# dog-qiuqiu/Yolo-FastestV2

Hardware: AMD Instinct MI355X
Metric: images/sec at 352x352 bs=256 per GPU (forward+decode+NMS) (higher is better)
Workload: dtype f32 tensors; contractions fp16x3 (two-term fp16 split operands on v_mfma_f32_16x16x32_f16, fp32 accumulate); depthwise/BN/ReLU/decode/NMS fp32 VALU; 1 GPU

## Files before the change

yolo_fastestv2_amd/csrc/yfv2_api.hip:

```cpp
#include <algorithm>
#include <cstdio>

#include "yfv2_ctx.h"

void read_plan_switches(yfv2_ctx* h, const yfv2_plan* plan) {
  h->sw.plan = read_sized(plan);
  h->sw.bf6 = !h->sw.plan.fp32_matrix;
  h->postfuse = !h->sw.plan.post_two_launches;
  h->sw.front_wanted = !h->sw.plan.front_two_launches;
}

int run_plan(yfv2_ctx* h, const void* x, bool x_u8, int B, float* const out6[6], hipStream_t stream, hipEvent_t* ev, int only_step) {
  const RunCtx c{h->d_params, x, x_u8, B, out6, stream, h->sw.bf6, h->nonfinite.dev};
  std::string err;
  if (int rc = plan_run(h->plan, c, h->d_trace, h->trace_step, ev, only_step, &err)) return fail(h, rc, err);
  if (only_step < 0) { h->last_x = x; h->last_B = B; h->last_u8 = x_u8; }
  HIP_TRY(h, hipGetLastError());
  return YFV2_OK;
}

int check_call(yfv2_ctx* h, int B, bool need_weights) {
  if (!h) return fail(nullptr, YFV2_ERR_ARG, "null handle");
  if (B < 1 || B > h->cfg.max_batch)
    return fail(h, YFV2_ERR_BATCH, "batch " + std::to_string(B) + " outside [1, max_batch=" + std::to_string(h->cfg.max_batch) + "]");
  if (need_weights && !h->weights_loaded) return fail(h, YFV2_ERR_STATE, "yfv2_load_weights has not been called");
  return YFV2_OK;
}

int check_config(const yfv2_config* cfg, int* rows_out) {
  if (cfg->anchor_num != 3)
    return fail(nullptr, YFV2_ERR_CONFIG, "anchor_num must be 3 (the reference decode hard-codes 3 anchors per scale)");
  if (cfg->classes < 1 || cfg->classes > 255)
    return fail(nullptr, YFV2_ERR_CONFIG, "classes must be in [1, 255]");
  if (cfg->height < 32 || cfg->width < 32 || cfg->height % 32 || cfg->width % 32)
    return fail(nullptr, YFV2_ERR_CONFIG, "height/width must be multiples of 32");
  if (cfg->max_batch < 1) return fail(nullptr, YFV2_ERR_CONFIG, "max_batch must be >= 1");
  const long long rows_ll = 3LL * ((long long)(cfg->height / 16) * (cfg->width / 16) + (long long)(cfg->height / 32) * (cfg->width / 32));
  if (rows_ll > yfv2_nms_max_rows())
    return fail(nullptr, YFV2_ERR_CONFIG, "more than " + std::to_string(yfv2_nms_max_rows()) + " decode rows per image (" + std::to_string(rows_ll) +
                                          ": inputs beyond 512x512) is not supported by the NMS kernel");
  const int rows = (int)rows_ll;
  *rows_out = rows;
  return YFV2_OK;
}

namespace {

thread_local std::string g_tls_error;
thread_local bool g_creating_lane = false;

int alloc_buf(yfv2_ctx* h, Buf* b, size_t per_img) {
  b->per_img = per_img;
  HIP_TRY(h, hipMalloc(reinterpret_cast<void**>(&b->p), per_img * sizeof(float) * (size_t)h->cfg.max_batch));
  return YFV2_OK;
}

void free_buf(Buf* b) {
  if (b->p) (void)hipFree(b->p);
  b->p = nullptr;
}

size_t logit_elems(const yfv2_ctx* h, int i) { return logit_elems(h->cfg, i); }

constexpr int LANES_DEFAULT = 1, LANES_MAX = 8, LANE_MIN_IMAGES = 32;

int create_lanes(yfv2_ctx* h) {
  int n = h->sw.plan.lanes > 1 ? h->sw.plan.lanes : LANES_DEFAULT;
  if (h->d_trace || h->in_lane) n = 1;
  n = n < 1 ? 1 : (n > LANES_MAX ? LANES_MAX : n);
  if (n == 1 || h->cfg.max_batch < n * LANE_MIN_IMAGES) return YFV2_OK;
  h->lane_min = n * LANE_MIN_IMAGES;
  yfv2_config c = h->cfg;
  c.max_batch = (h->cfg.max_batch + n - 1) / n;
  for (int i = 0; i < n; ++i) {
    yfv2_ctx* lane = nullptr;
    yfv2_plan lp = h->sw.plan;
    lp.lanes = 0; lp.trace = 0;
    g_creating_lane = true;
    const int rc = yfv2_create_ex(&lane, &c, &lp);
    g_creating_lane = false;
    if (rc) return fail(h, rc, "lane " + std::to_string(i) + ": " + g_tls_error);
    lane->nonfinite.dev = h->nonfinite.dev;
    h->lanes.push_back(lane);
  }
  HIP_TRY(h, hipEventCreateWithFlags(&h->lane_fork, hipEventDisableTiming));
  for (int i = 1; i < n; ++i) {
    hipStream_t st; hipEvent_t ev;
    HIP_TRY(h, hipStreamCreateWithFlags(&st, hipStreamNonBlocking));
    h->lane_stream.push_back(st);
    HIP_TRY(h, hipEventCreateWithFlags(&ev, hipEventDisableTiming));
    h->lane_join.push_back(ev);
  }
  return YFV2_OK;
}

template <class F>
int run_lanes(yfv2_ctx* h, int B, hipStream_t s, F f) {
  const int n = (int)h->lanes.size();
  const int per = (B + n - 1) / n;
  h->last_split.clear();
  h->last_x = nullptr; h->last_B = 0;
  HIP_TRY(h, hipEventRecord(h->lane_fork, s));
  int rc = YFV2_OK;
  auto hip_ok = [&](hipError_t e, const char* what) {
    if (e != hipSuccess && rc == YFV2_OK) rc = fail(h, YFV2_ERR_DEVICE, std::string(what) + ": " + hipGetErrorString(e));
    return e == hipSuccess;
  };
  std::vector<char> forked((size_t)n, 0);
  for (int i = 1; i < n && rc == YFV2_OK; ++i) {
    const int off = i * per, cnt = std::min(per, B - off);
    if (cnt <= 0) break;
    if (!hip_ok(hipStreamWaitEvent(h->lane_stream[i - 1], h->lane_fork, 0), "hipStreamWaitEvent(lane fork)")) break;
    forked[(size_t)i] = 1;
    const int lrc = f(h->lanes[i], off, cnt, h->lane_stream[i - 1]);
    if (lrc) { rc = lrc; h->err = h->lanes[i]->err; }
  }
  if (rc == YFV2_OK) {
    rc = f(h->lanes[0], 0, std::min(per, B), s);
    if (rc) h->err = h->lanes[0]->err;
  }
  for (int i = 1; i < n; ++i) {
    if (!forked[(size_t)i]) continue;
    if (hip_ok(hipEventRecord(h->lane_join[i - 1], h->lane_stream[i - 1]), "hipEventRecord(lane join)"))
      hip_ok(hipStreamWaitEvent(s, h->lane_join[i - 1], 0), "hipStreamWaitEvent(lane join)");
    else
      (void)hipStreamSynchronize(h->lane_stream[i - 1]);
  }
  if (rc == YFV2_OK)
    for (int i = 0; i < n; ++i) { const int cnt = std::min(per, B - i * per); if (cnt > 0) h->last_split.push_back(cnt); }
  return rc;
}

bool use_lanes(const yfv2_ctx* h, int B) { return !h->lanes.empty() && B >= h->lane_min; }

}

int build_plan(yfv2_ctx* h, WeightPacker& wp, const yfv2_tensor_desc* tensors, int32_t n, yfv2_ctx* report) {
  h->plan = Plan{};
  if (!wp.index(h->cfg, tensors, n)) return fail(report, YFV2_ERR_WEIGHTS, wp.missing);
  if (!plan_build(h->cfg, h->sw, h->ws, wp, &h->plan)) return fail(report, YFV2_ERR_WEIGHTS, "weight packing failed");
  return YFV2_OK;
}

void** yfv2_ctx_train_slot(yfv2_ctx* h) { return h ? &h->train : nullptr; }
const yfv2_config* yfv2_ctx_config(yfv2_ctx* h) { return &h->cfg; }
int yfv2_ctx_fail(yfv2_ctx* h, int code, const char* msg) {
  g_tls_error = msg ? msg : "";
  if (h) h->err = g_tls_error;
  return code;
}

DecodeArgs decode_args(yfv2_ctx* h, const float* const out6[6], int32_t B) {
  DecodeArgs a{};
  for (int sc = 0; sc < 2; ++sc) {
    a.reg[sc] = out6[sc * 3 + 0];
    a.obj[sc] = out6[sc * 3 + 1];
    a.cls[sc] = out6[sc * 3 + 2];
    a.fh[sc] = h->fh[sc];
    a.fw[sc] = h->fw[sc];
    a.stride[sc] = (float)((double)h->cfg.height / (double)h->fh[sc]);
  }
  for (int i = 0; i < 12; ++i) a.anchors[i] = h->cfg.anchors[i];
  a.B = B;
  a.classes = h->cfg.classes;
  a.rows = h->rows;
  return a;
}

NmsArgs nms_args(const yfv2_ctx* h, const float* boxes, int compact, int32_t B, float conf_thres, double iou_thres, float* dets, int32_t* idx, int32_t* count) {
  NmsArgs a{};
  a.boxes = boxes; a.compact = compact; a.dets = dets; a.idx = idx; a.count = count;
  a.B = B; a.rows = h->rows; a.nc = h->cfg.classes;
  a.conf_thres = conf_thres; a.iou_thres = iou_thres;
  return a;
}

static const void* image_at(const yfv2_ctx* h, const void* x, bool x_u8, int off) {
  return static_cast<const char*>(x) + (size_t)off * 3 * h->cfg.height * h->cfg.width * (x_u8 ? 1 : sizeof(float));
}

extern "C" {

int yfv2_abi_version(void) { return YFV2_ABI_VERSION; }

const char* yfv2_last_error(yfv2_handle h) { return h ? h->err.c_str() : g_tls_error.c_str(); }

int yfv2_create(yfv2_handle* out, const yfv2_config* cfg) { return yfv2_create_ex(out, cfg, nullptr); }

int yfv2_create_ex(yfv2_handle* out, const yfv2_config* cfg, const yfv2_plan* plan) {
  if (!out || !cfg) return fail(nullptr, YFV2_ERR_ARG, "yfv2_create: null argument");
  *out = nullptr;
  int rows = 0;
  if (int rc = check_config(cfg, &rows)) return rc;

  int ndev = 0;
  if (hipGetDeviceCount(&ndev) != hipSuccess || ndev <= 0 || cfg->device < 0 || cfg->device >= ndev)
    return fail(nullptr, YFV2_ERR_DEVICE, "no usable HIP device (this library has no CPU fallback)");
  hipDeviceProp_t prop;
  if (hipGetDeviceProperties(&prop, cfg->device) != hipSuccess)
    return fail(nullptr, YFV2_ERR_DEVICE, "hipGetDeviceProperties failed");
  if (std::strncmp(prop.gcnArchName, "gfx950", 6) != 0)
    return fail(nullptr, YFV2_ERR_DEVICE, std::string("device is ") + prop.gcnArchName + ", this library is built for gfx950 (MI355X) only");

  yfv2_ctx* h = new yfv2_ctx();
  h->in_lane = g_creating_lane;
  DeviceGuard guard(cfg->device);
  int rc = setup_ctx(h, cfg, rows, alloc_buf);
  if (rc == YFV2_OK && hipMalloc(reinterpret_cast<void**>(&h->d_classes), 258 * sizeof(int32_t)) != hipSuccess)
    rc = fail(h, YFV2_ERR_DEVICE, "hipMalloc(class filter) failed");
  if (rc == YFV2_OK && hipMalloc(reinterpret_cast<void**>(&h->d_frames), sizeof(ResizeFrame) * (size_t)cfg->max_batch) != hipSuccess)
    rc = fail(h, YFV2_ERR_DEVICE, "hipMalloc(frame table) failed");
  if (rc == YFV2_OK) {
    h->d_stats_flag = h->d_classes + 256;
    if (hipMemset(h->d_stats_flag, 0, 2 * sizeof(int32_t)) != hipSuccess) rc = fail(h, YFV2_ERR_DEVICE, "hipMemset(flags) failed");
  }
  if (rc == YFV2_OK && !h->in_lane) {
    if (!h->nonfinite.alloc()) rc = fail(h, YFV2_ERR_DEVICE, "hipHostMalloc(range-guard word) failed");
    else *reinterpret_cast<volatile int32_t*>(h->nonfinite.host) = 0;
  }
  if (rc != YFV2_OK) {
    g_tls_error = h->err;
    yfv2_destroy(h);
    return rc;
  }
  read_plan_switches(h, plan);
  if (h->sw.plan.trace) {
    h->trace_step = h->sw.plan.trace_step;
    (void)hipMalloc(reinterpret_cast<void**>(&h->d_trace), 8192 * sizeof(long long));
    (void)hipMemset(h->d_trace, 0, 8192 * sizeof(long long));
  }
  if (int rc2 = create_lanes(h)) { g_tls_error = h->err; yfv2_destroy(h); return rc2; }
  *out = h;
  return YFV2_OK;
}

void yfv2_destroy(yfv2_handle h) {
  if (!h) return;
  DeviceGuard guard(h->device);
  h->ws.for_each(h->cfg, h->rows, [](Buf& b, size_t) { free_buf(&b); });
  if (h->d_classes) (void)hipFree(h->d_classes);
  if (h->d_frames) (void)hipFree(h->d_frames);
  if (h->d_probe) (void)hipFree(h->d_probe);
  if (h->train) { yfv2_train_release(h->train); h->train = nullptr; }
  if (h->d_params) (void)hipFree(h->d_params);
  for (yfv2_ctx* lane : h->lanes) yfv2_destroy(lane);
  for (hipStream_t st : h->lane_stream) { (void)hipStreamSynchronize(st); (void)hipStreamDestroy(st); }
  for (hipEvent_t ev : h->lane_join) (void)hipEventDestroy(ev);
  if (h->lane_fork) (void)hipEventDestroy(h->lane_fork);
  delete h;
}

int yfv2_load_weights(yfv2_handle h, const yfv2_tensor_desc* tensors, int32_t n) {
  if (!h) return fail(nullptr, YFV2_ERR_ARG, "null handle");
  if (!tensors || n <= 0) return fail(h, YFV2_ERR_ARG, "yfv2_load_weights: no tensors");
  DeviceGuard guard(h->device);
  WeightPacker wp;
  if (int rc = build_plan(h, wp, tensors, n, h)) {
    h->weights_loaded = false;
    return rc;
  }
  HIP_TRY(h, hipDeviceSynchronize());
  if (h->d_params && h->n_params < wp.blob.size()) { (void)hipFree(h->d_params); h->d_params = nullptr; }
  if (!h->d_params) {
    HIP_TRY(h, hipMalloc(reinterpret_cast<void**>(&h->d_params), wp.blob.size() * sizeof(float)));
    h->n_params = wp.blob.size();
  }
  HIP_TRY(h, hipMemcpy(h->d_params, wp.blob.data(), wp.blob.size() * sizeof(float), hipMemcpyHostToDevice));
  h->weights_loaded = true;
  for (yfv2_ctx* lane : h->lanes)
    if (int rc = yfv2_load_weights(lane, tensors, n)) { h->weights_loaded = false; return fail(h, rc, lane->err); }
  return YFV2_OK;
}

int yfv2_set_anchors(yfv2_handle h, const double anchors[12]) {
  if (!h) return fail(nullptr, YFV2_ERR_ARG, "null handle");
  if (!anchors) return fail(h, YFV2_ERR_ARG, "yfv2_set_anchors: null pointer");
  for (int i = 0; i < 12; ++i) h->cfg.anchors[i] = anchors[i];
  for (yfv2_ctx* lane : h->lanes) (void)yfv2_set_anchors(lane, anchors);
  return YFV2_OK;
}

static int forward_impl(yfv2_handle h, const void* x, bool x_u8, int32_t B, float* const out6[6], void* stream) {
  const std::string name = x_u8 ? "yfv2_forward_u8" : "yfv2_forward";
  int rc = check_call(h, B, true);
  if (rc) return rc;
  if (!x || !out6) return fail(h, YFV2_ERR_ARG, name + ": null pointer");
  for (int i = 0; i < 6; ++i)
    if (!out6[i]) return fail(h, YFV2_ERR_ARG, name + ": null output tensor");
  DeviceGuard guard(h->device);
  if (use_lanes(h, B))
    return run_lanes(h, B, static_cast<hipStream_t>(stream), [&](yfv2_ctx* lane, int off, int cnt, hipStream_t st) {
      float* o6[6];
      for (int i = 0; i < 6; ++i) o6[i] = out6[i] + (size_t)off * logit_elems(h, i);
      return forward_impl(lane, image_at(h, x, x_u8, off), x_u8, cnt, o6, st);
    });
  h->last_split.clear();
  return run_plan(h, x, x_u8, B, out6, static_cast<hipStream_t>(stream), nullptr);
}
int yfv2_forward(yfv2_handle h, const float* x, int32_t B, float* const out6[6], void* stream) { return forward_impl(h, x, false, B, out6, stream); }
int yfv2_forward_u8(yfv2_handle h, const uint8_t* x, int32_t B, float* const out6[6], void* stream) { return forward_impl(h, x, true, B, out6, stream); }

static int post_impl(yfv2_handle h, const float* const out6[6], int32_t B, float conf_thres, double iou_thres, float* dets, int32_t* idx,
                     int32_t* count, void* stream);
static int decode_impl(yfv2_handle h, const float* const out6[6], int32_t B, float* boxes, float* cand, void* stream);
static int nms_impl(yfv2_handle h, const float* boxes, int compact, int32_t B, float conf_thres, double iou_thres,
                    const int32_t* classes, int32_t n_classes, float* dets, int32_t* idx, int32_t* count, void* stream);

int yfv2_decode(yfv2_handle h, const float* const out6[6], int32_t B, float* boxes, void* stream) {
  return decode_impl(h, out6, B, boxes, nullptr, stream);
}

static int decode_impl(yfv2_handle h, const float* const out6[6], int32_t B, float* boxes, float* cand, void* stream) {
  int rc = check_call(h, B, false);
  if (rc) return rc;
  if (!out6 || (!boxes && !cand)) return fail(h, YFV2_ERR_ARG, "yfv2_decode: null pointer");
  for (int i = 0; i < 6; ++i)
    if (!out6[i]) return fail(h, YFV2_ERR_ARG, "yfv2_decode: null logit tensor");
  DeviceGuard guard(h->device);
  DecodeArgs a = decode_args(h, out6, B);
  a.boxes = boxes;
  a.cand = cand;
  yfv2_launch_decode(a, static_cast<hipStream_t>(stream));
  HIP_TRY(h, hipGetLastError());
  return YFV2_OK;
}

// ... 121 lines not shown
```

yolo_fastestv2_amd/csrc/yfv2_internal.h:

```cpp
#pragma once
#include <hip/hip_runtime.h>
#include <hip/hip_ext.h>
#include <stdint.h>

typedef float f32x4 __attribute__((ext_vector_type(4)));
typedef float f32x2 __attribute__((ext_vector_type(2)));
typedef float f32x3u __attribute__((ext_vector_type(3), aligned(4)));
typedef unsigned int u32x2 __attribute__((ext_vector_type(2)));
typedef unsigned int u32x3 __attribute__((ext_vector_type(3)));

#ifdef __HIPCC__
__device__ __forceinline__ int yfv2_fdiv(int n, float inv_d) { return (int)(((float)n + 0.5f) * inv_d); }
#endif

#include <atomic>

struct Yfv2LaunchProbe { hipEvent_t start = nullptr, stop = nullptr; int launches = 0; };
extern thread_local Yfv2LaunchProbe yfv2_launch_probe;
#define YFV2_LAUNCH(kernel, grid, block, lds, stream, ...)                                                                        \
  do {                                                                                                                             \
    Yfv2LaunchProbe& yfv2_lp_ = yfv2_launch_probe;                                                                                 \
    hipExtLaunchKernelGGL(kernel, grid, block, lds, stream, yfv2_lp_.launches++ == 0 ? yfv2_lp_.start : nullptr, yfv2_lp_.stop, 0, \
                          __VA_ARGS__);                                                                                            \
  } while (0)
// ... 99 lines not shown
  int relu;
  float* copy;
  int copy_stride;
  int copy_off;
  int H, W;
  int HW;
  float* nchw0;
  float* nchw1;
  int split;
  int ctot0, coff0;
  int bf6;
  int presplit;
  int* nonfinite;
};

struct DwArgs {
  const float* in;
  float* out;
  const float* w;
  const float* scale;
  const float* shift;
  int B, H, W, C;
  int OH, OW;
  int in_stride, in_off;
  int out_stride, out_off;
  int relu;
};

struct BlockS1Args {
  const float* in;
  float* out;
  const float* img;
  long long* trace;
  int B, H, W;
  int R;
  int nblk;
  int presplit;
  int* nonfinite;
  float* park;
};

bool yfv2_s1chain_supported(int c2, int H, int W);
int yfv2_s1chain_image_floats();
long yfv2_s1chain_park_floats(int H, int W, int nblk);
bool yfv2_launch_block_s1chain(const BlockS1Args& a, hipStream_t s);
bool yfv2_s1pool_supported(int c2, int H, int W);
int yfv2_s1pool_image_floats(bool presplit);
bool yfv2_launch_block_s1pool(const BlockS1Args& a, hipStream_t s);

struct BlockS2Args {
  const float* in;
  float* out;
  const float* img;
  int B, H, W;
  int R;
  int s4_main_bands;
  int pp_in;
  unsigned pp_mask;
  long long pp_bufstride;
  long long pp_imgstride;
  int bf6;
  long long* trace;
  const float* img16;
  int* nonfinite;
};
bool yfv2_s3h_supported(int H, int W);
void yfv2_launch_s3h(const BlockS2Args& a, hipStream_t s);
bool yfv2_s4h_supported(int H, int W);
void yfv2_launch_s4h(const BlockS2Args& a, hipStream_t s);

__host__ __device__ inline int yfv2_stage2_channel(int slot) {
  const int p = slot >> 1, e = slot & 1;
  const int b0 = p / 12, b1 = (p % 12) / 6, b2 = (p % 6) / 3, h = 2 * (p % 3) + e;
  return b0 + 2 * b1 + 4 * b2 + 8 * h;
}
struct S1PxArgs {
  float* act;
  const float* img;
  int B, H, W;
  int nstrips, nb, R;
  int img_stride;
  int num_records;
  int src_off[12];
  int dst_off[12];
  const float* img16;
  int* nonfinite;
};
struct S2PxArgs {
  const float* in;
  float* act;
  const float* img[2];
  int B, IH, IW;
  int nstrips, nb, R;
  int in_stride, out_stride;
  int in_records, out_records;
  int st2_off[2][8];
  int st1_off[2][8];
  const float* img16;
  int* nonfinite;
};
struct FrontArgs {
  const void* x;
  int H, W;
  int u8_in;
  const float* img_stem;
  S2PxArgs s2;
};
void yfv2_launch_front(const FrontArgs& a, hipStream_t s);
void yfv2_launch_s2px(const S2PxArgs& a, hipStream_t s);
void yfv2_launch_s2h(const S2PxArgs& a, hipStream_t s);
bool yfv2_s1px_supported(int H, int W);
void yfv2_launch_s1px(const S1PxArgs& a, hipStream_t s);
void yfv2_launch_s1h(const S1PxArgs& a, hipStream_t s);

struct TowerArgs {
  const float* in;
  float* out;
  const float* img;
  int has_head;
  int mh, split;
  float* nchw0; float* nchw1;
  int B, H, W;
  long long* trace;
  int bf6;
  const float* img16;
  int chain;
  int* nonfinite;
};

struct DecodeArgs {
  const float* reg[2];
  const float* obj[2];
  const float* cls[2];
  float* boxes;
  float* cand;
  int B, classes;
  int fh[2], fw[2];
  float stride[2];
  double anchors[12];
  int rows;
};

struct NmsArgs {
  const float* boxes;
  int compact;
  float* dets;
  int32_t* idx;
  int32_t* count;
  const int32_t* classes;
  int n_classes;
  int B, rows, nc;
  float conf_thres;
  double iou_thres;
  long long* trace;
};

void yfv2_launch_stem(const StemArgs& a, hipStream_t s);
void yfv2_launch_stem16(const StemArgs& a, hipStream_t s);
bool yfv2_launch_pw(int K, int mode, const PwArgs& a, hipStream_t s);
int yfv2_pw_tiles(int K, int mode, int M);
bool yfv2_pw_presplit_supported(int K, int mode, int M);
bool yfv2_launch_dw(int ksize, int stride, const DwArgs& a, hipStream_t s);
int yfv2_block_s2_rows(int cin, int H, int W);
bool yfv2_launch_block_s2(int cin, const BlockS2Args& a, hipStream_t s);
bool yfv2_tower2_supported(int H, int W);
bool yfv2_launch_tower2(const TowerArgs& a, hipStream_t s);
bool yfv2_towerh_supported(int H, int W);
bool yfv2_towerh_multi(int H, int W);
struct TowerJobs {
  TowerArgs j[4];
  int n;
  int par;
  int gpj;
  unsigned char lane_patch[128];
};
bool yfv2_launch_towerh(const TowerJobs& jobs, int mh_tiles, hipStream_t s);
struct StatsArgs {
  const float* dets;
  const int32_t* count;
  const float* targets;
  int32_t* tp;
  int32_t* overflow;
  int B, T;
  float iou_thres;
};
constexpr int STATS_MAX_TARGETS = 1024;
void yfv2_launch_stats(const StatsArgs& a, hipStream_t s);
struct StatsMultiArgs {
  const float* dets; const int32_t* count; const float* targets;
  uint32_t* tpmask;
  int32_t* overflow;
  int B, T, K;
  float thr[32];
};
void yfv2_launch_stats_multi(const StatsMultiArgs& a, hipStream_t s);
struct LossMatch {
  int valid, b, a, gj, gi, cls;
  float tb[4];
  double aw, ah;
};
struct LossArgs {
  const float* reg[2]; const float* obj[2]; const float* cls[2];
  float* grad_reg[2]; float* grad_obj[2]; float* grad_cls[2];
  const float* targets;
  LossMatch* matches;
  unsigned char* tobj[2];
  int* nb;
  double* sums;
  float* losses;
  int B, T, classes;
  int fh[2], fw[2];
  double stride[2];
  double anchors[12];
};
void yfv2_launch_loss(const LossArgs& a, hipStream_t s);
struct ResizeArgs {
  const unsigned char* src;
  unsigned char* dst;
  int B, SH, SW, H, W;
  double scale_x, scale_y;
};
size_t yfv2_resize_lds_bytes(int SW, int W);
void yfv2_launch_resize(const ResizeArgs& a, hipStream_t s);
struct ResizeFrame {
  const unsigned char* data;
  long long pitch;
  int h, w;
  double scale_x, scale_y;
  double box_x, box_y;
};
void yfv2_launch_resize_frames(const ResizeFrame* frames, int B, int max_w, unsigned char* dst, int H, int W, hipStream_t s);
void yfv2_launch_frame_boxes(float* dets, const int32_t* count, const ResizeFrame* frames, int B, hipStream_t s);
void yfv2_launch_decode(const DecodeArgs& a, hipStream_t s);
void yfv2_launch_nms(const NmsArgs& a, hipStream_t s);
void yfv2_launch_decode_nms(const DecodeArgs& d, const NmsArgs& a, hipStream_t s);
bool yfv2_post_fusable(int classes, int rows);
int yfv2_nms_max_rows();
struct TileMergeArgs {
  const float* tile_dets;
  const int32_t* tile_count;
  const int32_t* table;
  int T, F;
  float* geo;
  float* meta;
  double thres;
  int metric;
  int max_out;
  float* dets;
  int32_t* src;
  int32_t* count;
};
void yfv2_launch_tile_merge(const TileMergeArgs& a, hipStream_t s);
constexpr int YFV2_KM_CH = 1024;
constexpr int YFV2_KM_MAXK = 32;
struct KmArgs {
  const double* wh;
  int64_t N;
  double* centroids;
  int k;
  int64_t nchunks;
  int32_t* assign;
  double* avg_iou;
  double* part_sum;
  int* part_cnt;
  int* part_flag;
  int* done;
  int32_t* host_word;
};
void yfv2_launch_km_pass(const KmArgs& a, int pass, int last, hipStream_t s);
constexpr int YFV2_AP_CH = 1024;
constexpr int YFV2_AP_TILE = 2048;
struct ApHead {
  long long n_gt[256], n_pred[256];
  double p[256], r[256], ap[256];
  int32_t bad, pad;
};
struct ApArgs {
  const int32_t* tp; const float* conf; const float* pred_cls;
  const uint32_t* tpmask;
  int K;
  int64_t N;
  const float* target_cls;
  int64_t T;
  uint32_t* key[2];
  uint32_t* val[2];
  uint32_t* hist;
  uint32_t* tot;
  double* part;
  int64_t part_stride;
  uint32_t* pmask;
  ApHead* head;
  int nblk;
};
size_t yfv2_ap_ws_bytes(int64_t N, int K);
void yfv2_ap_carve(ApArgs& a, char* ws);
void yfv2_launch_ap(const ApArgs& a, hipStream_t s);
struct yfv2_ap_result;
void yfv2_ap_finish(const ApHead& head, yfv2_ap_result* out);
void yfv2_ap_finish_multi(ApHead* heads, int K, yfv2_ap_result* out);
struct ClockProbeArgs {
  unsigned long long* out;
  unsigned long long ref_ticks;
  int busy;
};
bool yfv2_launch_clock_probe(const ClockProbeArgs& a, int workgroups, hipStream_t s);

struct yfv2_ctx;
struct yfv2_config;
// ... 5 lines not shown
```

yolo_fastestv2_amd/csrc/yfv2_post.hip:

```cpp
#include "yfv2_internal.h"

__device__ __forceinline__ float sigmoid_f32(float x) { return __fdiv_rn(1.0f, __fadd_rn(1.0f, expf(-x))); }

template <int J>
__device__ __forceinline__ int quad_xor(int v) {
  static_assert(J == 1 || J == 2, "quad_perm exchange inside four lanes");
  return __builtin_amdgcn_update_dpp(0, v, J == 1 ? 0xB1 : 0x4E, 0xF, 0xF, false);
}
template <int J> __device__ __forceinline__ float quad_xor(float v) { return __int_as_float(quad_xor<J>(__float_as_int(v))); }

template <bool SKIP = false, int MAXPER = 24>
__device__ __forceinline__ void yfv2_compact_row(const DecodeArgs& a, int b, int sc, int cc, int part, f32x4& r0, f32x4& r1,
                                                 float objl = 0.f, float skip_ct = 0.f) {
  const int fh = a.fh[sc], fw = a.fw[sc], hw = fh * fw;
  const int nc = a.classes;
  const int per = (nc + 3) >> 2;
  const int c_lo = part * per, c_hi = min(nc, c_lo + per);
  const int an = part < 3 ? part : 0;
  const float* cls = a.cls[sc] + (size_t)b * nc * hw;
  const float so = sigmoid_f32(SKIP ? objl : a.obj[sc][((size_t)b * 3 + an) * hw + cc]);
  float conf = 0.f;
  int cj = 0;
  int need = 1;
  if constexpr (SKIP) {
// ... 176 lines not shown
        if (c < c_hi) {
          srow[5 + c] = ev[i];
          srow[rowlen + 5 + c] = ev[i];
          srow[2 * rowlen + 5 + c] = ev[i];
        }
      }
      if (part < 3) {
        float o[5];
        box_of(part, o);
        float* d = srow + part * rowlen;
#pragma unroll
        for (int k = 0; k < 5; ++k) d[k] = o[k];
      }
    }
    __syncthreads();
    float* dst = a.boxes + row0 * rowlen;
    const int n = ncell * 3 * rowlen;
    for (int i = tid; i < n; i += THREADS) dst[i] = stage[i];
  }
}

void yfv2_launch_decode(const DecodeArgs& a, hipStream_t s) {
  const int cells = a.classes <= 96 ? DEC_CELLS : 32;
  const int b0 = (a.fh[0] * a.fw[0] + cells - 1) / cells;
  const int b1 = (a.fh[1] * a.fw[1] + cells - 1) / cells;
  const size_t lds = (size_t)cells * 3 * (5 + a.classes) * sizeof(float);
  static std::atomic<unsigned long long> lds_ok0{0}, lds_ok1{0}, lds_ok2{0}, lds_ok3{0};
  if (a.classes <= 96) {
    yfv2_allow_full_lds(reinterpret_cast<const void*>(&decode_kernel<false>), lds_ok0);
    yfv2_allow_full_lds(reinterpret_cast<const void*>(&decode_kernel<true>), lds_ok1);
    if (a.cand)
      YFV2_LAUNCH(decode_kernel<true>, dim3(a.B * (b0 + b1)), dim3(DEC_THREADS), 0, s, a, b0, b1);
    else
      YFV2_LAUNCH(decode_kernel<false>, dim3(a.B * (b0 + b1)), dim3(DEC_THREADS), lds, s, a, b0, b1);
  } else {
    yfv2_allow_full_lds(reinterpret_cast<const void*>(&decode_kernel<false, 64>), lds_ok2);
    yfv2_allow_full_lds(reinterpret_cast<const void*>(&decode_kernel<true, 64>), lds_ok3);
    if (a.cand)
      YFV2_LAUNCH((decode_kernel<true, 64>), dim3(a.B * (b0 + b1)), dim3(4 * cells), 0, s, a, b0, b1);
    else
      YFV2_LAUNCH((decode_kernel<false, 64>), dim3(a.B * (b0 + b1)), dim3(4 * cells), lds, s, a, b0, b1);
  }
}
bool yfv2_post_fusable(int classes, int rows) { return classes <= 96 && rows <= 2048; }
int yfv2_nms_max_rows() { return 4096; }

constexpr int NMS_THREADS = 1024;
constexpr int NMS_NQ = NMS_THREADS / 64;
constexpr int NMS_CAP = 2048;
constexpr int NMS_MAX_DET = 300;

__device__ __forceinline__ unsigned xor_sel_mask() {
  const int l = (int)(threadIdx.x & 63);
  const bool s4 = __builtin_amdgcn_update_dpp(0, l, 0x124, 0xF, 0xF, false) == (l ^ 4);
  const auto p16 = __builtin_amdgcn_permlane16_swap(l, l, false, false);
  const auto p32 = __builtin_amdgcn_permlane32_swap(l, l, false, false);
  return (s4 ? 4u : 0u) | ((int)p16[0] == (l ^ 16) ? 16u : 0u) | ((int)p32[0] == (l ^ 32) ? 32u : 0u);
}
template <int J>
__device__ __forceinline__ unsigned xor_lane32(unsigned v, unsigned sel) {
  const int x = (int)v;
  if constexpr (J == 1 || J == 2) return (unsigned)quad_xor<J>(x);
  else if constexpr (J == 8) return (unsigned)__builtin_amdgcn_update_dpp(0, x, 0x128, 0xF, 0xF, false);
  else if constexpr (J == 4) {
    const int r4 = __builtin_amdgcn_update_dpp(0, x, 0x124, 0xF, 0xF, false), r12 = __builtin_amdgcn_update_dpp(0, x, 0x12C, 0xF, 0xF, false);
    return (unsigned)((sel & 4u) ? r4 : r12);
  } else if constexpr (J == 16) {
    const auto p = __builtin_amdgcn_permlane16_swap(x, x, false, false);
    return (unsigned)((sel & 16u) ? (int)p[0] : (int)p[1]);
  } else {
    static_assert(J == 32, "lane distance");
    const auto p = __builtin_amdgcn_permlane32_swap(x, x, false, false);
    return (unsigned)((sel & 32u) ? (int)p[0] : (int)p[1]);
  }
}
template <int J>
__device__ __forceinline__ unsigned long long xor_lane64(unsigned long long v, unsigned sel) {
  return ((unsigned long long)xor_lane32<J>((unsigned)(v >> 32), sel) << 32) | xor_lane32<J>((unsigned)v, sel);
}

template <int KPT>
__device__ __forceinline__ void bitonic_sort(unsigned long long* key, unsigned long long* key2, int np2, int tid) {
  const unsigned sel = xor_sel_mask();
  unsigned long long k[KPT];
#pragma unroll
  for (int r = 0; r < KPT; ++r) { const int i = tid + r * NMS_THREADS; k[r] = i < np2 ? key[i] : 0ull; }
  auto cx = [](unsigned long long x, unsigned long long y, bool take_max) { return take_max == (x > y) ? x : y; };
  int pb = 0;
  for (int kk = 2; kk <= np2; kk <<= 1) {
    int j = kk >> 1;
    for (; j >= 64; j >>= 1) {
      if (j >= NMS_THREADS) {
        const int jr = j / NMS_THREADS;
#pragma unroll
        for (int r = 0; r < KPT; ++r) {
          if ((r & jr) == 0 && (r | jr) < KPT) {
            const int r2 = r | jr;
            const bool desc = ((tid + r * NMS_THREADS) & kk) == 0;
            const unsigned long long hi = k[r] > k[r2] ? k[r] : k[r2], lo = k[r] > k[r2] ? k[r2] : k[r];
            k[r] = desc ? hi : lo; k[r2] = desc ? lo : hi;
          }
        }
      } else {
        unsigned long long* buf = pb ? key2 : key;
#pragma unroll
        for (int r = 0; r < KPT; ++r) buf[tid + r * NMS_THREADS] = k[r];
        __syncthreads();
        const bool low = (tid & j) == 0;
#pragma unroll
        for (int r = 0; r < KPT; ++r) {
          const int i = tid + r * NMS_THREADS;
          k[r] = cx(k[r], buf[i ^ j], low == ((i & kk) == 0));
        }
        pb ^= 1;
      }
    }
#define YFV2_SORT_STEP(J)                                                                   \
    if (J < kk) {                                                                           \
      const bool low = (tid & J) == 0;                                                      \
      _Pragma("unroll") for (int r = 0; r < KPT; ++r) {                                     \
        const int i = tid + r * NMS_THREADS;                                                \
        k[r] = cx(k[r], xor_lane64<J>(k[r], sel), low == ((i & kk) == 0));                 \
      }                                                                                     \
    }
    YFV2_SORT_STEP(32) YFV2_SORT_STEP(16) YFV2_SORT_STEP(8) YFV2_SORT_STEP(4) YFV2_SORT_STEP(2) YFV2_SORT_STEP(1)
#undef YFV2_SORT_STEP
  }
  __syncthreads();
#pragma unroll
  for (int r = 0; r < KPT; ++r) { const int i = tid + r * NMS_THREADS; if (i < np2) key[i] = k[r]; }
  __syncthreads();
}

__device__ __forceinline__ unsigned conf_key(float c) {
  const unsigned u = __float_as_uint(c == 0.f ? 0.f : c);
  return (u & 0x80000000u) ? ~u : (u | 0x80000000u);
}

#define NMS_STAMP(i) do { if (a.trace && blockIdx.x == 0 && threadIdx.x == 0) a.trace[i] = (long long)__builtin_readcyclecounter(); } while (0)
template <int SRC, int KPT = 2>
__global__ __launch_bounds__(NMS_THREADS) void nms_kernel(NmsArgs a, DecodeArgs dec) {
  constexpr bool COMPACT = SRC >= 1;
  constexpr int CAP = KPT * NMS_THREADS;
  static_assert(KPT == 2 || (KPT == 4 && SRC != 2), "two keys per thread, or four without the in-LDS decode");
  extern __shared__ __attribute__((aligned(16))) float crow[];
  __shared__ unsigned long long key[CAP];
  __shared__ __attribute__((aligned(16))) float geo[(KPT == 2 ? 7 : 5) * CAP];
  unsigned long long* const key2 = reinterpret_cast<unsigned long long*>(geo);
  float* const bx1 = geo + (KPT == 2 ? 2 * CAP : 0);
  float* const by1 = bx1 + CAP; float* const bx2 = by1 + CAP; float* const by2 = bx2 + CAP; float* const area = by2 + CAP;
  __shared__ unsigned char supp[CAP];
  __shared__ unsigned char cls_of_row[CAP];
  __shared__ int keep[NMS_MAX_DET];
  __shared__ float kx1[NMS_MAX_DET], kx2[NMS_MAX_DET];
  __shared__ unsigned long long pmask[NMS_NQ][64];
  __shared__ int n_cand, n_keep, n_obj;

  const int tid = threadIdx.x, b = blockIdx.x;
  const int rowlen = COMPACT ? 8 : 5 + a.nc;
  const float* img = SRC == 2 ? crow : a.boxes + (size_t)b * a.rows * rowlen;
  const float ct = a.conf_thres;
  NMS_STAMP(0);
  if constexpr (SRC == 2) {
    constexpr int WC = 16;
    const int hw0 = dec.fh[0] * dec.fw[0], hw1 = dec.fh[1] * dec.fw[1];
    const int nw0 = (hw0 + WC - 1) / WC, nw = nw0 + (hw1 + WC - 1) / WC;
    const int wv = __builtin_amdgcn_readfirstlane(tid >> 6);
    const int part = tid & 3, an = part < 3 ? part : 0;
    auto obj_of = [&](int w) -> float {
      if (w >= nw) return 0.f;
      const int sc = w >= nw0 ? 1 : 0, hw = sc ? hw1 : hw0;
      const int cell = (w - (sc ? nw0 : 0)) * WC + ((tid & 63) >> 2);
      return dec.obj[sc][((size_t)b * 3 + an) * hw + (cell < hw ? cell : hw - 1)];
    };
    float ocur = obj_of(wv);
    for (int w = wv; w < nw; w += NMS_NQ) {
      const float onxt = obj_of(w + NMS_NQ);
      const int sc = w >= nw0 ? 1 : 0, hw = sc ? hw1 : hw0;
      const int row_base = sc ? 3 * hw0 : 0;
      const int cell = (w - (sc ? nw0 : 0)) * WC + ((tid & 63) >> 2);
      const bool ok = cell < hw;
      f32x4 r0, r1;
      yfv2_compact_row<true>(dec, b, sc, ok ? cell : hw - 1, part, r0, r1, ocur, ct);
      if (ok && part < 3) {
        float* d = crow + (size_t)(row_base + cell * 3 + part) * 8;
        *reinterpret_cast<f32x4*>(d) = r0;
        *reinterpret_cast<f32x4*>(d + 4) = r1;
      }
      ocur = onxt;
    }
    __syncthreads();
  }
  NMS_STAMP(1);
  unsigned short* cand_row = reinterpret_cast<unsigned short*>(bx1);
  if (tid == 0) { n_cand = 0; n_keep = 0; n_obj = 0; }
  __syncthreads();

  if constexpr (COMPACT) {
    for (int n0 = 0; n0 < a.rows; n0 += NMS_THREADS) {
      const int n = n0 + tid;
      f32x4 t = {0.f, 0.f, 0.f, 0.f};
      if (n < a.rows) t = *reinterpret_cast<const f32x4*>(img + (size_t)n * 8 + 4);
      const bool pass = n < a.rows && t[0] > ct && t[1] > ct;
      const unsigned long long m = __ballot(pass);
      int base = 0;
      if ((tid & 63) == 0 && m) base = atomicAdd(&n_cand, (int)__popcll(m));
      base = __shfl(base, 0);
      if (pass) {
        const int slot = base + (int)__popcll(m & ((1ull << (tid & 63)) - 1ull));
        key[slot] = ((unsigned long long)conf_key(t[1]) << 32) | (unsigned long long)(0xFFFFFFFFu - (unsigned)n);
        cls_of_row[n] = (unsigned char)(int)t[2];
      }
    }
  } else {
    for (int n0 = 0; n0 < a.rows; n0 += NMS_THREADS) {
      const int n = n0 + tid;
      const bool pass = n < a.rows && img[(size_t)n * rowlen + 4] > ct;
      const unsigned long long m = __ballot(pass);
      int base = 0;
      if ((tid & 63) == 0 && m) base = atomicAdd(&n_obj, (int)__popcll(m));
      base = __shfl(base, 0);
      if (pass) cand_row[base + (int)__popcll(m & ((1ull << (tid & 63)) - 1ull))] = (unsigned short)n;
    }
    __syncthreads();
    {
      const int l16 = tid & 15, grp = tid >> 4, ngrp = NMS_THREADS >> 4;
      const int nobj = n_obj;
      for (int q = grp; q < nobj; q += ngrp) {
        const int n = cand_row[q];
        const float* r = img + (size_t)n * rowlen;
        const float obj = r[4];
        float best = -INFINITY;
        int bj = 0x7fffffff;
        for (int j = l16; j < a.nc; j += 16) {
          const float pj = __fmul_rn(r[5 + j], obj);
          if (pj > best || (pj != pj && best == best)) { best = pj; bj = j; }
        }
#pragma unroll
        for (int m = 1; m < 16; m <<= 1) {
          const float ob = __shfl_xor(best, m, 16);
          const int oj = __shfl_xor(bj, m, 16);
          const bool take = ob != ob ? (best == best || oj < bj) : (best == best && (ob > best || (ob == best && oj < bj)));
          if (take) { best = ob; bj = oj; }
        }
        if (l16 == 0 && best > ct) {
          bool hit = true;
          if (a.classes) {
            hit = false;
            for (int k = 0; k < a.n_classes; ++k) hit |= (a.classes[k] == bj);
          }
          if (hit) {
            const int slot = atomicAdd(&n_cand, 1);
            key[slot] = ((unsigned long long)conf_key(best) << 32) | (unsigned long long)(0xFFFFFFFFu - (unsigned)n);
            cls_of_row[n] = (unsigned char)bj;
          }
        }
      }
    }
  }
  __syncthreads();
  NMS_STAMP(2);
  const int n = n_cand;
  if (n == 0) {
    if (tid == 0) a.count[b] = 0;
    return;
  }

  int np2 = 1;
  while (np2 < n) np2 <<= 1;
  for (int i = n + tid; i < np2; i += NMS_THREADS) key[i] = 0ull;
  __syncthreads();
  if (np2 <= NMS_THREADS) bitonic_sort<1>(key, key2, np2, tid);
  else bitonic_sort<KPT>(key, key2, np2, tid);

  NMS_STAMP(3);
  for (int i = tid; i < n; i += NMS_THREADS) {
    const unsigned row = 0xFFFFFFFFu - (unsigned)(key[i] & 0xFFFFFFFFull);
    const float* r = img + (size_t)row * rowlen;
    const float cx = r[0], cy = r[1], hw_ = __fdiv_rn(r[2], 2.0f), hh = __fdiv_rn(r[3], 2.0f);
    const float c = __fmul_rn((float)cls_of_row[row], 4096.0f);
    const float x1 = __fadd_rn(__fsub_rn(cx, hw_), c), y1 = __fadd_rn(__fsub_rn(cy, hh), c);
    const float x2 = __fadd_rn(__fadd_rn(cx, hw_), c), y2 = __fadd_rn(__fadd_rn(cy, hh), c);
    bx1[i] = x1; by1[i] = y1; bx2[i] = x2; by2[i] = y2;
    area[i] = __fmul_rn(__fsub_rn(x2, x1), __fsub_rn(y2, y1));
    supp[i] = 0;
  }
  __syncthreads();

  NMS_STAMP(4);
  const bool thr_nonneg = a.iou_thres >= 0.0;
  auto overlaps = [&](int i, int j) -> bool {
    const float xx1 = fmaxf(bx1[i], bx1[j]), xx2 = fminf(bx2[i], bx2[j]);
    if (thr_nonneg && !(xx2 > xx1)) return false;
    const float yy1 = fmaxf(by1[i], by1[j]), yy2 = fminf(by2[i], by2[j]);
    const float w = fmaxf(0.0f, __fsub_rn(xx2, xx1)), h = fmaxf(0.0f, __fsub_rn(yy2, yy1));
    const float inter = __fmul_rn(w, h);
    const float ovr = __fdiv_rn(inter, __fsub_rn(__fadd_rn(area[i], area[j]), inter));
    return (double)ovr > a.iou_thres;
  };
  const int j = tid & 63, q = tid >> 6;
  long long t_tests = 0, t_walk = 0, t_bar = 0; int n_chunks = 0;
  const bool tr = a.trace && blockIdx.x == 0 && tid == 0;
  for (int c0 = 0; c0 < n; c0 += 64) {
    const int nk = n_keep;
    if (nk >= NMS_MAX_DET) break;
    const long long ts0 = tr ? (long long)__builtin_readcyclecounter() : 0;
    const int m = min(64, n - c0);
    unsigned long long bits = 0ull;
    {
      constexpr int KMAX = (NMS_MAX_DET + NMS_NQ - 1) / NMS_NQ;
      constexpr int PER = 64 / NMS_NQ;
      auto lane_f = [](float v, int l) { return __builtin_bit_cast(float, __builtin_amdgcn_readlane(__builtin_bit_cast(int, v), l)); };
      const int cj = c0 + j;
      const bool live = j < m;
      const float jx1 = live ? bx1[cj] : INFINITY, jx2 = live ? bx2[cj] : -INFINITY;
      const int kl = q + NMS_NQ * j;
      const bool kv = j < KMAX && kl < nk;
      const float rk1 = kv ? kx1[kl] : INFINITY, rk2 = kv ? kx2[kl] : -INFINITY;
      unsigned cand = 0u;
#pragma unroll
      for (int t = 0; t < KMAX; ++t) {
        const float a1 = lane_f(rk1, t), a2 = lane_f(rk2, t);
        if (q + NMS_NQ * t < nk && (!thr_nonneg || fminf(a2, jx2) > fmaxf(a1, jx1))) cand |= 1u << t;
      }
      unsigned icand = 0u;
#pragma unroll
      for (int c = 0; c < PER; ++c) {
        const int i = PER * q + c;
        const float a1 = lane_f(jx1, i), a2 = lane_f(jx2, i);
        if (i < j && (!thr_nonneg || fminf(a2, jx2) > fmaxf(a1, jx1))) icand |= 1u << c;
      }
      if (live) {
        while (cand) {
          const int t = __builtin_ctz(cand);
          cand &= cand - 1u;
          if (overlaps(keep[q + NMS_NQ * t], cj)) { supp[cj] = 1; break; }
        }
        while (icand) {
          const int c = __builtin_ctz(icand);
          icand &= icand - 1u;
          if (overlaps(c0 + PER * q + c, cj)) bits |= 1ull << (PER * q + c);
        }
      }
    }
    pmask[q][j] = bits;
    const long long ts1 = tr ? (long long)__builtin_readcyclecounter() : 0;
    __syncthreads();
    const long long ts2 = tr ? (long long)__builtin_readcyclecounter() : 0;
    if (tid < 64) {
      unsigned long long S = 0ull;
#pragma unroll
      for (int qq = 0; qq < NMS_NQ; ++qq) S |= pmask[qq][tid];
      const bool alive = tid < m && !supp[c0 + tid];
      const unsigned long long alive_mask = __ballot(alive);
      unsigned long long kmask = alive_mask;
      for (int it = 0; it < 64; ++it) {
        const unsigned long long k2 = __ballot(alive && !(S & kmask));
        if (k2 == kmask) break;
        kmask = k2;
      }
      if ((kmask >> tid) & 1ull) {
        const int pos = nk + __popcll(kmask & ((1ull << tid) - 1ull));
        if (pos < NMS_MAX_DET) { keep[pos] = c0 + tid; kx1[pos] = bx1[c0 + tid]; kx2[pos] = bx2[c0 + tid]; }
      }
      if (tid == 0) n_keep = min(NMS_MAX_DET, nk + __popcll(kmask));
    }
    const long long ts3 = tr ? (long long)__builtin_readcyclecounter() : 0;
    __syncthreads();
    if (tr) { const long long ts4 = (long long)__builtin_readcyclecounter(); t_tests += ts1 - ts0; t_walk += ts3 - ts2; t_bar += (ts2 - ts1) + (ts4 - ts3); ++n_chunks; }
  }
  if (tr) { a.trace[9] = n_chunks; a.trace[10] = t_tests; a.trace[11] = t_walk; a.trace[12] = t_bar; }
  __syncthreads();
  NMS_STAMP(5);
  const int kept = n_keep;

  for (int k = tid; k < kept; k += NMS_THREADS) {
    const int i = keep[k];
    const unsigned long long kk = key[i];
    const unsigned row = 0xFFFFFFFFu - (unsigned)(kk & 0xFFFFFFFFull);
    const float* r = img + (size_t)row * rowlen;
    const float cx = r[0], cy = r[1], hw_ = __fdiv_rn(r[2], 2.0f), hh = __fdiv_rn(r[3], 2.0f);
    float* d = a.dets + ((size_t)b * NMS_MAX_DET + k) * 6;
    d[0] = __fsub_rn(cx, hw_); d[1] = __fsub_rn(cy, hh);
    d[2] = __fadd_rn(cx, hw_); d[3] = __fadd_rn(cy, hh);
    d[4] = COMPACT ? r[5] : __fmul_rn(r[5 + cls_of_row[row]], r[4]);
    d[5] = (float)cls_of_row[row];
    a.idx[(size_t)b * NMS_MAX_DET + k] = (int)row;
  }
  if (tid == 0) a.count[b] = kept;
  NMS_STAMP(6);
  if (a.trace && blockIdx.x == 0 && tid == 0) { a.trace[7] = n; a.trace[8] = kept; }
}

void yfv2_launch_nms(const NmsArgs& a, hipStream_t s) {
  const DecodeArgs none{};
  if (a.rows <= NMS_CAP) {
    if (a.compact)
      YFV2_LAUNCH(nms_kernel<1>, dim3(a.B), dim3(NMS_THREADS), 0, s, a, none);
    else
      YFV2_LAUNCH(nms_kernel<0>, dim3(a.B), dim3(NMS_THREADS), 0, s, a, none);
  } else {
    if (a.compact)
      YFV2_LAUNCH((nms_kernel<1, 4>), dim3(a.B), dim3(NMS_THREADS), 0, s, a, none);
    else
      YFV2_LAUNCH((nms_kernel<0, 4>), dim3(a.B), dim3(NMS_THREADS), 0, s, a, none);
  }
}

void yfv2_launch_decode_nms(const DecodeArgs& d, const NmsArgs& a, hipStream_t s) {
  static std::atomic<unsigned long long> done{0};
  int dev = 0;
  if (hipGetDevice(&dev) != hipSuccess || dev < 0 || dev > 63) dev = 0;
  if (!(done.load() & (1ull << dev))) {
    (void)hipFuncSetAttribute(reinterpret_cast<const void*>(&nms_kernel<2>), hipFuncAttributeMaxDynamicSharedMemorySize, NMS_CAP * 8 * (int)sizeof(float));
    done.fetch_or(1ull << dev);
  }
  YFV2_LAUNCH(nms_kernel<2>, dim3(a.B), dim3(NMS_THREADS), (size_t)a.rows * 8 * sizeof(float), s, a, d);
}

__device__ __forceinline__ int stats_load_targets(const float* __restrict__ targets, int T, int b, int lane, float* tx1, float* ty1, float* tx2,
                                                  float* ty2, float* tlab) {
  int nt = 0;
  for (int t0 = 0; t0 < T; t0 += 64) {
    const int t = t0 + lane;
    const bool mine = t < T && targets[(size_t)t * 6] == (float)b;
    const unsigned long long m = __ballot(mine);
    if (mine) {
      const int pos = nt + __popcll(m & ((1ull << lane) - 1ull));
      if (pos < STATS_MAX_TARGETS) {
        tlab[pos] = targets[(size_t)t * 6 + 1];
        tx1[pos] = targets[(size_t)t * 6 + 2]; ty1[pos] = targets[(size_t)t * 6 + 3];
        tx2[pos] = targets[(size_t)t * 6 + 4]; ty2[pos] = targets[(size_t)t * 6 + 5];
      }
    }
    nt += __popcll(m);
  }
  return nt;
}

__device__ __forceinline__ void stats_best_scan(const float* __restrict__ d, int nt, int lane, const float* tx1, const float* ty1, const float* tx2,
                                                const float* ty2, const float* tlab, bool& has, float& best, int& bidx) {
  const float bx1 = d[0], by1 = d[1], bx2 = d[2], by2 = d[3], lab = d[5];
  const float barea = __fmul_rn(__fadd_rn(__fsub_rn(bx2, bx1), 1.f), __fadd_rn(__fsub_rn(by2, by1), 1.f));
  has = false;
  best = -1.f;
  bidx = 0x7fffffff;
  for (int t = lane; t < nt; t += 64) {
    has |= tlab[t] == lab;
    const float ix1 = fmaxf(bx1, tx1[t]), iy1 = fmaxf(by1, ty1[t]), ix2 = fminf(bx2, tx2[t]), iy2 = fminf(by2, ty2[t]);
    const float iw = fmaxf(__fadd_rn(__fsub_rn(ix2, ix1), 1.f), 0.f), ih = fmaxf(__fadd_rn(__fsub_rn(iy2, iy1), 1.f), 0.f);
    const float inter = __fmul_rn(iw, ih);
    const float tarea = __fmul_rn(__fadd_rn(__fsub_rn(tx2[t], tx1[t]), 1.f), __fadd_rn(__fsub_rn(ty2[t], ty1[t]), 1.f));
    const float iou = __fdiv_rn(inter, __fadd_rn(__fsub_rn(__fadd_rn(barea, tarea), inter), 1e-16f));
    if (iou > best) { best = iou; bidx = t; }
  }
}

__device__ __forceinline__ void stats_best_reduce(float& best, int& bidx) {
#pragma unroll
  for (int off = 32; off > 0; off >>= 1) {
    const float ob = __shfl_xor(best, off);
    const int oi = __shfl_xor(bidx, off);
    if (ob > best || (ob == best && oi < bidx)) { best = ob; bidx = oi; }
  }
}

__global__ __launch_bounds__(64) void stats_kernel(StatsArgs a) {
  __shared__ float tx1[STATS_MAX_TARGETS], ty1[STATS_MAX_TARGETS], tx2[STATS_MAX_TARGETS], ty2[STATS_MAX_TARGETS], tlab[STATS_MAX_TARGETS];
  __shared__ int tdone[STATS_MAX_TARGETS];
  const int b = blockIdx.x, lane = threadIdx.x;
  int nt = stats_load_targets(a.targets, a.T, b, lane, tx1, ty1, tx2, ty2, tlab);
  if (nt > STATS_MAX_TARGETS) { if (lane == 0) *a.overflow = 1; nt = STATS_MAX_TARGETS; }
  for (int t = lane; t < nt; t += 64) tdone[t] = 0;
  __syncthreads();
  const int n = a.count[b];
  int* tp = a.tp + (size_t)b * NMS_MAX_DET;
  for (int i = lane; i < NMS_MAX_DET; i += 64) tp[i] = 0;
  if (nt == 0) return;
  const float thr = a.iou_thres;
  int matched = 0;
  for (int i = 0; i < n && matched < nt; ++i) {
    bool has;
    float best;
    int bidx;
    stats_best_scan(a.dets + ((size_t)b * NMS_MAX_DET + i) * 6, nt, lane, tx1, ty1, tx2, ty2, tlab, has, best, bidx);
    if (__ballot(has) == 0ull) continue;
    stats_best_reduce(best, bidx);
    if (best >= thr && tdone[bidx] == 0) {
      if (lane == 0) { tp[i] = 1; tdone[bidx] = 1; }
      ++matched;
    }
    __syncthreads();
  }
}

constexpr int STATSM_WAVES = 8;
__global__ __launch_bounds__(64 * STATSM_WAVES) void stats_multi_kernel(StatsMultiArgs a) {
  __shared__ float tx1[STATS_MAX_TARGETS], ty1[STATS_MAX_TARGETS], tx2[STATS_MAX_TARGETS], ty2[STATS_MAX_TARGETS], tlab[STATS_MAX_TARGETS];
  __shared__ unsigned tdone[STATS_MAX_TARGETS];
  __shared__ float s_best[NMS_MAX_DET];
  __shared__ int s_bidx[NMS_MAX_DET];
  __shared__ float s_thr[32];
  __shared__ int s_nt;
  const int b = blockIdx.x, tid = threadIdx.x, lane = tid & 63, wave = tid >> 6;
  if (wave == 0) {
    const int all = stats_load_targets(a.targets, a.T, b, lane, tx1, ty1, tx2, ty2, tlab);
    if (lane == 0) {
      if (all > STATS_MAX_TARGETS) *a.overflow = 1;
      s_nt = all > STATS_MAX_TARGETS ? STATS_MAX_TARGETS : all;
    }
  } else if (wave == 1) {
    if (lane < 32) s_thr[lane] = lane < a.K ? a.thr[lane] : __builtin_nanf("");
  }
  for (int t = tid; t < STATS_MAX_TARGETS; t += 64 * STATSM_WAVES) tdone[t] = 0u;
  __syncthreads();
  const int nt = s_nt;
// ... 57 lines not shown
```

Measured before the change: 469,100 images/s.

## Vectorize NMS IoU tests with wave-wide ballots and a float fast-path threshold

Restructures the NMS chunk loop so that each pairwise overlap test is evaluated across the whole wavefront with readlane/ballot instead of per-lane serial candidate walks. It adds an fp32 IoU threshold comparison (inter - T*denom against an error margin) that settles most pairs without the exact division and double compare, falling back to the exact overlaps() only for ambiguous pairs. Kept boxes now also store y coordinates and area in LDS. This is meant to cut divergent per-lane loops and the division cost, but it adds more LDS state and a subtle rounding-margin argument that must preserve exact results.

```diff
diff --git a/yolo_fastestv2_amd/csrc/yfv2_api.hip b/yolo_fastestv2_amd/csrc/yfv2_api.hip
--- a/yolo_fastestv2_amd/csrc/yfv2_api.hip
+++ b/yolo_fastestv2_amd/csrc/yfv2_api.hip
@@ -172,6 +172,7 @@
   a.boxes = boxes; a.compact = compact; a.dets = dets; a.idx = idx; a.count = count;
   a.B = B; a.rows = h->rows; a.nc = h->cfg.classes;
   a.conf_thres = conf_thres; a.iou_thres = iou_thres;
+  a.iou_fast = nms_iou_threshold_f32(iou_thres, &a.iou_T) ? 1 : 0;
   return a;
 }
 
diff --git a/yolo_fastestv2_amd/csrc/yfv2_internal.h b/yolo_fastestv2_amd/csrc/yfv2_internal.h
--- a/yolo_fastestv2_amd/csrc/yfv2_internal.h
+++ b/yolo_fastestv2_amd/csrc/yfv2_internal.h
@@ -275,8 +275,19 @@
   int B, rows, nc;
   float conf_thres;
   double iou_thres;
+  float iou_T;
+  int iou_fast;
   long long* trace;
 };
+
+inline bool nms_iou_threshold_f32(double thr, float* T) {
+  if (thr != thr) { *T = NAN; return false; }
+  float f = (float)thr;
+  if (!((double)f > thr)) f = nextafterf(f, INFINITY);
+  else { const float g = nextafterf(f, -INFINITY); if ((double)g > thr) f = g; }
+  *T = f;
+  return thr >= 0.0 && thr < 1.0 && f >= 0x1p-20f;
+}
 
 void yfv2_launch_stem(const StemArgs& a, hipStream_t s);
 void yfv2_launch_stem16(const StemArgs& a, hipStream_t s);
diff --git a/yolo_fastestv2_amd/csrc/yfv2_post.hip b/yolo_fastestv2_amd/csrc/yfv2_post.hip
--- a/yolo_fastestv2_amd/csrc/yfv2_post.hip
+++ b/yolo_fastestv2_amd/csrc/yfv2_post.hip
@@ -352,7 +352,7 @@
   __shared__ unsigned char supp[CAP];
   __shared__ unsigned char cls_of_row[CAP];
   __shared__ int keep[NMS_MAX_DET];
-  __shared__ float kx1[NMS_MAX_DET], kx2[NMS_MAX_DET];
+  __shared__ float kx1[NMS_MAX_DET], kx2[NMS_MAX_DET], ky1[NMS_MAX_DET], ky2[NMS_MAX_DET], karea[NMS_MAX_DET];
   __shared__ unsigned long long pmask[NMS_NQ][64];
   __shared__ int n_cand, n_keep, n_obj;
 
@@ -498,49 +498,67 @@
     const float ovr = __fdiv_rn(inter, __fsub_rn(__fadd_rn(area[i], area[j]), inter));
     return (double)ovr > a.iou_thres;
   };
-  const int j = tid & 63, q = tid >> 6;
+  const float iouT = a.iou_T, iouT2 = a.iou_T * 0x1p-21f;
+  const bool fast = a.iou_fast != 0;
+  const int j = tid & 63, q = __builtin_amdgcn_readfirstlane(tid >> 6);
   long long t_tests = 0, t_walk = 0, t_bar = 0; int n_chunks = 0;
   const bool tr = a.trace && blockIdx.x == 0 && tid == 0;
   for (int c0 = 0; c0 < n; c0 += 64) {
-    const int nk = n_keep;
+    const int nk = __builtin_amdgcn_readfirstlane(n_keep);
     if (nk >= NMS_MAX_DET) break;
     const long long ts0 = tr ? (long long)__builtin_readcyclecounter() : 0;
     const int m = min(64, n - c0);
     unsigned long long bits = 0ull;
+    const int cj = c0 + j;
+    const bool live = j < m;
+    const float jx1 = __builtin_canonicalizef(live ? bx1[cj] : INFINITY), jx2 = __builtin_canonicalizef(live ? bx2[cj] : -INFINITY);
+    const float jy1 = __builtin_canonicalizef(live ? by1[cj] : INFINITY), jy2 = __builtin_canonicalizef(live ? by2[cj] : -INFINITY);
+    const float ja = live ? area[cj] : 0.f;
     {
-      constexpr int KMAX = (NMS_MAX_DET + NMS_NQ - 1) / NMS_NQ;
       constexpr int PER = 64 / NMS_NQ;
-      auto lane_f = [](float v, int l) { return __builtin_bit_cast(float, __builtin_amdgcn_readlane(__builtin_bit_cast(int, v), l)); };
-      const int cj = c0 + j;
-      const bool live = j < m;
-      const float jx1 = live ? bx1[cj] : INFINITY, jx2 = live ? bx2[cj] : -INFINITY;
+      const unsigned long long any_x = thr_nonneg ? 0ull : ~0ull;
+      auto lane_i = [](float v, int l) { return __builtin_amdgcn_readlane(__builtin_bit_cast(int, v), l); };
+      auto was_max = [](int s, float v) { float r; asm("v_max_f32 %0, %1, %2" : "=v"(r) : "s"(s), "v"(v)); return r; };
+      auto was_min = [](int s, float v) { float r; asm("v_min_f32 %0, %1, %2" : "=v"(r) : "s"(s), "v"(v)); return r; };
+      auto pair = [&](float sx1, float sx2, float sy1, float sy2, float sa, int so, int l, unsigned long long on) -> unsigned long long {
+        const float xx1 = was_max(lane_i(sx1, l), jx1), xx2 = was_min(lane_i(sx2, l), jx2);
+        const unsigned long long pre = on & (__builtin_amdgcn_ballot_w64(xx2 > xx1) | any_x);
+        if (!pre) return 0ull;
+        unsigned long long yes = 0ull, amb = pre;
+        if (fast) {
+          const float yy1 = was_max(lane_i(sy1, l), jy1), yy2 = was_min(lane_i(sy2, l), jy2);
+          const float w = __fsub_rn(xx2, xx1);
+          const float h = fmaxf(0.0f, __fsub_rn(yy2, yy1));
+          const float inter = __fmul_rn(w, h);
+          const float denom = __fsub_rn(__fadd_rn(__builtin_bit_cast(float, lane_i(sa, l)), ja), inter);
+          const float d = __fmaf_rn(-iouT, denom, inter), e = __fmul_rn(denom, iouT2);
+          const unsigned long long ok = __builtin_amdgcn_ballot_w64(denom >= 0x1p-80f);
+          yes = pre & ok & __builtin_amdgcn_ballot_w64(d > e);
+          amb = pre & ~(ok & __builtin_amdgcn_ballot_w64(fabsf(d) > e));
+        }
+        if (amb) {
+          const int oi = __builtin_amdgcn_readlane(so, l);
+          bool r = false;
+          if ((amb >> j) & 1ull) r = overlaps(oi, cj);
+          yes |= __builtin_amdgcn_ballot_w64(r);
+        }
+        return yes;
+      };
+      const unsigned long long live_m = __builtin_amdgcn_ballot_w64(live);
+      const int nt = (nk - q + NMS_NQ - 1) / NMS_NQ;
       const int kl = q + NMS_NQ * j;
-      const bool kv = j < KMAX && kl < nk;
-      const float rk1 = kv ? kx1[kl] : INFINITY, rk2 = kv ? kx2[kl] : -INFINITY;
-      unsigned cand = 0u;
-#pragma unroll
-      for (int t = 0; t < KMAX; ++t) {
-        const float a1 = lane_f(rk1, t), a2 = lane_f(rk2, t);
-        if (q + NMS_NQ * t < nk && (!thr_nonneg || fminf(a2, jx2) > fmaxf(a1, jx1))) cand |= 1u << t;
-      }
-      unsigned icand = 0u;
+      const bool kv = j < nt;
+      const float rx1 = kv ? kx1[kl] : INFINITY, rx2 = kv ? kx2[kl] : -INFINITY;
+      const float ry1 = kv ? ky1[kl] : INFINITY, ry2 = kv ? ky2[kl] : -INFINITY, ra = kv ? karea[kl] : 0.f;
+      const int rkeep = kv ? keep[kl] : 0;
+      unsigned long long sup = 0ull;
+      for (int t = 0; t < nt; ++t) sup |= pair(rx1, rx2, ry1, ry2, ra, rkeep, t, live_m);
+      if ((sup >> j) & 1ull) supp[cj] = 1;
 #pragma unroll
       for (int c = 0; c < PER; ++c) {
         const int i = PER * q + c;
-        const float a1 = lane_f(jx1, i), a2 = lane_f(jx2, i);
-        if (i < j && (!thr_nonneg || fminf(a2, jx2) > fmaxf(a1, jx1))) icand |= 1u << c;
-      }
-      if (live) {
-        while (cand) {
-          const int t = __builtin_ctz(cand);
-          cand &= cand - 1u;
-          if (overlaps(keep[q + NMS_NQ * t], cj)) { supp[cj] = 1; break; }
-        }
-        while (icand) {
-          const int c = __builtin_ctz(icand);
-          icand &= icand - 1u;
-          if (overlaps(c0 + PER * q + c, cj)) bits |= 1ull << (PER * q + c);
-        }
+        const unsigned long long s = pair(jx1, jx2, jy1, jy2, ja, cj, i, live_m & ~((2ull << i) - 1ull));
+        bits |= ((s >> j) & 1ull) << i;
       }
     }
     pmask[q][j] = bits;
@@ -561,7 +579,7 @@
       }
       if ((kmask >> tid) & 1ull) {
         const int pos = nk + __popcll(kmask & ((1ull << tid) - 1ull));
-        if (pos < NMS_MAX_DET) { keep[pos] = c0 + tid; kx1[pos] = bx1[c0 + tid]; kx2[pos] = bx2[c0 + tid]; }
+        if (pos < NMS_MAX_DET) { keep[pos] = cj; kx1[pos] = jx1; kx2[pos] = jx2; ky1[pos] = jy1; ky2[pos] = jy2; karea[pos] = ja; }
       }
       if (tid == 0) n_keep = min(NMS_MAX_DET, nk + __popcll(kmask));
     }
```

After: 473,500 images/s (median of 6 runs). About the same (+0.9%).
